# wuxiyang1996/iPLAN

Hardware: AMD Instinct MI355X
Metric: env-steps/sec (whole node), Hetero-Highway chaotic 5-agent (higher is better)
Workload: dtype f32; 1 GPU; Highway chaotic full iPLAN (Behaviour + GAT + soft update), 5 agents x 55 entities, 32 envs/GPU x 90 steps; step = 8 rollouts, each followed by insert + Behavior_policy.learn + Prediction_policy.learn, then IPPOLearner.train (15 epochs x 255 x 90 rows x 5 agents); envs_per_gpu=32

## Files before the change

### iplan_amd/csrc/ac_fwd_body.h

```cpp
#pragma once
#include "api_util.h"
#include "gru_tile.h"
#include "ac_kmap.h"

namespace iplan {

__device__ __forceinline__ f32x4 ac_act4(f32x4 v, bool tanh) {
    f32x4 r;
    for (int q = 0; q < 4; ++q) r[q] = tanh ? tanh_f(v[q]) : (v[q] > 0.0f ? v[q] : 0.0f);
    return r;
}

constexpr int AM = IPLAN_AC_HIDDEN;
constexpr int AT = AM / 16;
#ifndef AC_RT
#define AC_RT 2
#endif


template <int RT, int NW = 8>
struct AcShared {
#ifdef AC_NO_STAGED_TAIL
    static constexpr bool STAGED_BUILD = false, STAGED2 = false;
#else
    static constexpr bool STAGED_BUILD = RT == 1, STAGED2 = RT == 2;
#endif
    static constexpr int TLDW = AM + 8;
    static constexpr int TW_ROWS = STAGED2 ? AM + 3 * AM + 16 + 3 * AM : (STAGED_BUILD ? AM + 3 * AM + 16 : 0);
    static constexpr int TP_FLOATS = 912;
    float red[NW][16], red2[NW][16], cc[NW][2][AM];
    float hand[4];
    __attribute__((aligned(16))) f32x4 acc[RT == 1 ? 8 : 1][AT][64];
    __attribute__((aligned(16))) float tw[TW_ROWS ? TW_ROWS * TLDW : 4];
    __attribute__((aligned(16))) f32x4 gh[STAGED_BUILD ? 3 * AT : 1][64];
    __attribute__((aligned(16))) float tp[TW_ROWS ? TP_FLOATS : 4];
};

struct AcGrid {
    int bx, by, bz, gx, gy, gz;
};

struct AcProducers {
    int32_t* sync;
    int n_prod, n_cons;
};

__device__ __forceinline__ void ac_signal_producer_done(int32_t* sync) {
#ifdef IPLAN_HOST_EMULATION
    __syncthreads();
    if (threadIdx.x == 0) sync[0] += 1;
#else
    asm volatile("s_waitcnt vmcnt(0)" ::: "memory");
    __syncthreads();
    if (threadIdx.x == 0) {
#if IPLAN_FUSED_FENCES
        __builtin_amdgcn_fence(__ATOMIC_RELEASE, "agent");
#endif
        __hip_atomic_fetch_add(sync, 1, __ATOMIC_RELAXED, __HIP_MEMORY_SCOPE_AGENT);
    }
#endif
}

__device__ __forceinline__ void ac_wait_producers(const AcProducers& pr) {
#ifdef IPLAN_HOST_EMULATION
    if (threadIdx.x == 0) {
        if (pr.sync[0] < pr.n_prod) pr.sync[2] = 1;
        if (++pr.sync[1] == pr.n_cons) { pr.sync[0] = 0; pr.sync[1] = 0; }
    }
    __syncthreads();
#else
    if (threadIdx.x == 0) {
        int spins = 0;
        while (__hip_atomic_load(pr.sync, __ATOMIC_RELAXED, __HIP_MEMORY_SCOPE_AGENT) < pr.n_prod) {
            __builtin_amdgcn_s_sleep(2);
            if (++spins > (1 << 22)) { __hip_atomic_store(pr.sync + 2, 1, __ATOMIC_RELAXED, __HIP_MEMORY_SCOPE_AGENT); break; }
        }
#if IPLAN_FUSED_FENCES
        __builtin_amdgcn_fence(__ATOMIC_ACQUIRE, "agent");
#endif
        if (__hip_atomic_fetch_add(pr.sync + 1, 1, __ATOMIC_RELAXED, __HIP_MEMORY_SCOPE_AGENT) == pr.n_cons - 1) {
            __hip_atomic_store(pr.sync + 1, 0, __ATOMIC_RELAXED, __HIP_MEMORY_SCOPE_AGENT);
            __hip_atomic_store(pr.sync, 0, __ATOMIC_RELAXED, __HIP_MEMORY_SCOPE_AGENT);
        }
    }
    __syncthreads();
    asm volatile("" ::: "memory");
#endif
}

template <int RT, bool PRE, bool FUSED, int NW = 8>
__device__ __forceinline__ void ac_fwd_body(const IplanAcFwdArgs& a, const AcGrid& gp, AcShared<RT, NW>& sh, const AcProducers& prod) {
    auto& s_red = sh.red;
    auto& s_red2 = sh.red2;
    auto& s_cc = sh.cc;
    auto& s_acc = sh.acc;
    constexpr int TLDW = AM + 8;
#ifdef AC_NO_STAGED_TAIL
    constexpr bool STAGED_BUILD = false, STAGED2 = false;
#else
    constexpr bool STAGED_BUILD = RT == 1, STAGED2 = RT == 2;
#endif
    constexpr int TW_ROWS = AcShared<RT, NW>::TW_ROWS;
    static_assert(TLDW == AcShared<RT, NW>::TLDW, "tail weight row stride");
    auto& s_tw = sh.tw;
    auto& s_gh = sh.gh;
    constexpr int TP_FC1B = 0, TP_LN1W = 64, TP_LN1B = 128, TP_FC2B = 192, TP_LN2W = 256, TP_LN2B = 320, TP_BIH = 384, TP_BHH = 576,
                  TP_LN3W = 768, TP_LN3B = 832, TP_HEADB = 896, TP_FLOATS = 912;
    static_assert(TP_FLOATS == AcShared<RT, NW>::TP_FLOATS, "tail parameter vectors");
    auto& s_tp = sh.tp;

    int bx = gp.bx, by = gp.by, bz = gp.bz;
#ifndef AC_NO_XCD_REMAP
    {
        const int X = gp.gx, G = X * gp.gy * gp.gz;
        const int b = bx + X * (by + gp.gy * bz);
        const int k = b & 7, slot = b >> 3, q8 = G >> 3, r8 = G & 7;
        const int item = k * q8 + (k < r8 ? k : r8) + slot;
        bx = item % X;
        const int pair = item / X;
        by = pair % gp.gy;
        bz = pair / gp.gy;
    }
#endif
    const int net = by;
    const int which = a.which == 2 ? bz : a.which;
    const IplanAcNet& nw = which ? a.critic : a.actor;
    const float* __restrict__ P = nw.params + (int64_t)net * nw.params_s_net;
    const IplanAcFeatures& ft = a.feat;
    const int l = lane_id(), w = uniform_i(wave_id()), n = l & 15, g = l >> 4;
    const int ks = RT == 1 ? a.ksplit : 1;
    const int groups = NW / ks;
    const int part = w % ks;
    const int KW = (RT == 1 && !PRE && a.ksplit_wg > 1 && ks == 8) ? a.ksplit_wg : 1;
    const int pw = bx % KW;
    bx /= KW;
    const int kpart = part * KW + pw;
    const bool clk = !FUSED && a.phase_clocks && bx == 0 && by == 0 && bz == 0 && threadIdx.x == 0;
    if (clk) a.phase_clocks[0] = IPLAN_CLOCK();
    int64_t* fclk = (FUSED && a.phase_clocks && threadIdx.x == 0) ? a.phase_clocks + 8 * (gp.bx + gp.gx * (gp.by + gp.gy * gp.bz)) : nullptr;
    if (fclk) fclk[0] = IPLAN_CLOCK();
    const KMap km = make_kmap(ft);
    const int F = km.NW + km.n_actions + km.n_id;
    const int KT = km.kt0[4];
    const float* __restrict__ pkw = which ? a.packed_critic : a.packed_actor;
    if (pkw) pkw += (int64_t)net * a.packed_s_net;
    const float* __restrict__ pkg = pkw ? pkw + (int64_t)KT * 1024 : nullptr;
    const float* __restrict__ pkb = pkw ? pkg + (int64_t)KT * 16 : nullptr;
    const float* __restrict__ pkc = pkw ? pkb + (int64_t)KT * 16 : nullptr;
    const int T_lo = kpart, T_hi = KT, T_st = ks * KW;

    int rr[RT], last[RT];
    bool vld[RT];
    int64_t prr[RT];
    const float* src[RT][3];
    for (int t = 0; t < RT; ++t) {
        const int tile = (bx * groups + w / ks) * RT + t;
        rr[t] = tile * 16 + n;
        vld[t] = rr[t] < a.rows;
        prr[t] = vld[t] ? (int64_t)(rr[t] / ft.T) * ft.T_phys + (rr[t] % ft.T) : 0;
        for (int s = 0; s < 3; ++s)
            src[t][s] = ft.w[s] > 0 ? ft.src[s] + (int64_t)net * ft.s_net[s] + prr[t] * ft.s_row[s] : nullptr;
        last[t] = -1;
        if (vld[t] && ft.n_actions > 0) {
            if (ft.last_action) last[t] = ft.last_action[(int64_t)net * ft.la_s_net + prr[t] * ft.la_s_row];
            else if (ft.last_action64) last[t] = (int)ft.last_action64[(int64_t)net * ft.la64_s_net + prr[t] * ft.la64_s_row];
        }
    }

    const bool staged = STAGED_BUILD && ks == 8 && groups == 1 && a.saved == nullptr;
    if (STAGED_BUILD && staged) {
        const float* Wsrc[3] = {P + nw.off[IPLAN_AC_FC2_W], P + nw.off[IPLAN_AC_WIH], P + nw.off[IPLAN_AC_HEAD_W]};
        for (int c = (int)threadIdx.x; c < (AM + 3 * AM + 16) * 16; c += 64 * NW) {
            const int r = c >> 4, c4 = c & 15;
            f32x4 v = splat4(0.f);
            if (r < AM) v = *reinterpret_cast<const f32x4*>(Wsrc[0] + r * AM + 4 * c4);
            else if (r < 4 * AM) v = *reinterpret_cast<const f32x4*>(Wsrc[1] + (r - AM) * AM + 4 * c4);
            else if (r - 4 * AM < nw.n_out) v = *reinterpret_cast<const f32x4*>(Wsrc[2] + (r - 4 * AM) * AM + 4 * c4);
            *reinterpret_cast<f32x4*>(&s_tw[r * TLDW + 4 * c4]) = v;
        }
        const float* hsrc0 = which ? a.h_critic : a.h_actor;
        const float* hrow0 = hsrc0 + (int64_t)net * a.hs_net + prr[0] * a.hs_row;
        f32x4 h0[AT];
        for (int t = 0; t < AT; ++t) h0[t] = vload(hrow0, vld[0], AM, t);
        for (int t = w; t < 3 * AT; t += NW)
            s_gh[t][l] = dense_tile_ga<AT>(P + nw.off[IPLAN_AC_WHH], AM, 3 * AM, 16 * t, h0, bfrag_a(P + nw.off[IPLAN_AC_BHH], t));
    }

    if (STAGED2) {
        const float* Wsrc[4] = {P + nw.off[IPLAN_AC_FC2_W], P + nw.off[IPLAN_AC_WIH], P + nw.off[IPLAN_AC_HEAD_W], P + nw.off[IPLAN_AC_WHH]};
        for (int c = (int)threadIdx.x; c < TW_ROWS * 16; c += 64 * NW) {
            const int r = c >> 4, c4 = c & 15;
            f32x4 v = splat4(0.f);
            if (r < AM) v = *reinterpret_cast<const f32x4*>(Wsrc[0] + r * AM + 4 * c4);
            else if (r < 4 * AM) v = *reinterpret_cast<const f32x4*>(Wsrc[1] + (r - AM) * AM + 4 * c4);
            else if (r < 4 * AM + 16) { if (r - 4 * AM < nw.n_out) v = *reinterpret_cast<const f32x4*>(Wsrc[2] + (r - 4 * AM) * AM + 4 * c4); }
            else v = *reinterpret_cast<const f32x4*>(Wsrc[3] + (r - 4 * AM - 16) * AM + 4 * c4);
            *reinterpret_cast<f32x4*>(&s_tw[r * TLDW + 4 * c4]) = v;
        }
    }

    const bool lds_tail = STAGED2 || (STAGED_BUILD && staged);
    if (TW_ROWS && lds_tail) {
        const int tp_off[11] = {TP_FC1B, TP_LN1W, TP_LN1B, TP_FC2B, TP_LN2W, TP_LN2B, TP_BIH, TP_BHH, TP_LN3W, TP_LN3B, TP_HEADB};
        const int tp_src[11] = {IPLAN_AC_FC1_B, IPLAN_AC_LN1_W, IPLAN_AC_LN1_B, IPLAN_AC_FC2_B, IPLAN_AC_LN2_W, IPLAN_AC_LN2_B, IPLAN_AC_BIH,
                                IPLAN_AC_BHH, IPLAN_AC_LN3_W, IPLAN_AC_LN3_B, IPLAN_AC_HEAD_B};
#pragma unroll
        for (int k = 0; k < 11; ++k) {
            const int len = k == 10 ? 16 : ((k == 6 || k == 7) ? 3 * AM : AM), have = k == 10 ? nw.n_out : len;
            for (int i = (int)threadIdx.x; i < len; i += 64 * NW) s_tp[tp_off[k] + i] = i < have ? P[nw.off[tp_src[k]] + i] : 0.f;
        }
    }

    const bool fold = !PRE && RT == 1 && ks > 1 && a.ln_stats_mode == 0;
    float mu[RT], rstd[RT];
    float fsx = 0.f, fsxx = 0.f;
    float c1a[AT], c2a[AT];
    for (int o = 0; o < AT; ++o) { c1a[o] = 0.f; c2a[o] = 0.f; }
    if (fold) {
        for (int t = 0; t < RT; ++t) { mu[t] = 0.f; rstd[t] = 1.f; }
    } else if (PRE || a.ln_stats_mode == 2) {
        for (int t = 0; t < RT; ++t) {
            mu[t] = 0.f; rstd[t] = 0.f;
            if (vld[t]) {
                const float* st = a.ln_stats + (int64_t)net * a.ln_stats_s_net + prr[t] * 2;
                mu[t] = st[0]; rstd[t] = st[1];
            }
        }
    } else {
        float s[RT];
        for (int t = 0; t < RT; ++t) s[t] = 0.f;
        for (int T = T_lo; T < T_hi; T += T_st) {
            const KTile kt = ktile(km, T);
            for (int t = 0; t < RT; ++t) {
                const f32x4 x = kfeat<FUSED>(km, kt, src[t], vld[t], last[t], net);
                s[t] += (x[0] + x[1]) + (x[2] + x[3]);
            }
        }
        for (int t = 0; t < RT; ++t) s[t] = group_sum(s[t]);
        if (ks > 1) {
            if (g == 0) s_red[w][n] = s[0];
            __syncthreads();
            float m = 0.f;
            for (int p2 = 0; p2 < ks; ++p2) m += s_red[(w / ks) * ks + p2][n];
            s[0] = m;
            __syncthreads();
        }
        for (int t = 0; t < RT; ++t) mu[t] = s[t] / (float)F;
        float v2[RT];
        for (int t = 0; t < RT; ++t) v2[t] = 0.f;
        for (int T = T_lo; T < T_hi; T += T_st) {
            const KTile kt = ktile(km, T);
            for (int t = 0; t < RT; ++t) {
                const f32x4 x = kfeat<FUSED>(km, kt, src[t], vld[t], last[t], net);
                for (int q = 0; q < 4; ++q)
                    if (q < kt.nv) { const float d = x[q] - mu[t]; v2[t] = fmaf(d, d, v2[t]); }
            }
        }
        for (int t = 0; t < RT; ++t) v2[t] = group_sum(v2[t]);
        if (ks > 1) {
            if (g == 0) s_red[w][n] = v2[0];
            __syncthreads();
            float m = 0.f;
            for (int p2 = 0; p2 < ks; ++p2) m += s_red[(w / ks) * ks + p2][n];
            v2[0] = m;
        }
        for (int t = 0; t < RT; ++t) {
            rstd[t] = 1.0f / sqrtf(v2[t] / (float)F + 1e-5f);
            if (a.ln_stats_mode == 1 && vld[t] && g == 0 && part == 0) {
                float* st = a.ln_stats + (int64_t)net * a.ln_stats_s_net + prr[t] * 2;
                st[0] = mu[t]; st[1] = rstd[t];
            }
        }
    }

    if (clk) a.phase_clocks[1] = IPLAN_CLOCK();
    const float* fnw = P + nw.off[IPLAN_AC_FN_W];
    const float* fnb = P + nw.off[IPLAN_AC_FN_B];
    const float* W1 = P + nw.off[IPLAN_AC_FC1_W];
    f32x4 accs[RT][AT];
    for (int t = 0; t < RT; ++t)
        for (int o = 0; o < AT; ++o) accs[t][o] = splat4(0.f);
#ifdef AC_NO_GROUPS
    constexpr bool GROUPED = false;
#else
    constexpr bool GROUPED = !PRE && RT > 1;
#endif
    f32x4 blk[GROUPED ? RT : 1][GROUPED ? AT : 1];
    if (GROUPED)
        for (int t = 0; t < RT; ++t)
            for (int o = 0; o < AT; ++o) blk[GROUPED ? t : 0][GROUPED ? o : 0] = splat4(0.f);
    auto flush_group = [&]() {
        if constexpr (GROUPED)
            for (int t = 0; t < RT; ++t)
                for (int o = 0; o < AT; ++o) { accs[t][o] += blk[t][o]; blk[t][o] = splat4(0.f); }
    };
    auto acc_mma = [&](const f32x4& wfrag, const f32x4& xfrag, int t, int oo) {
        if constexpr (GROUPED) blk[t][oo] = mma_block(wfrag, xfrag, blk[t][oo]);
        else accs[t][oo] = mma_block(wfrag, xfrag, accs[t][oo]);
    };
    struct KOps {
        KTile kt;
        f32x4 gm, bt, x[RT], wf[AT];
    };
    auto kload = [&](int T, KOps& o) {
        o.kt = ktile(km, T);
        for (int t = 0; t < RT; ++t) o.x[t] = kfeat<FUSED>(km, o.kt, src[t], vld[t], last[t], net);
        if (pkw) {
            o.gm = *reinterpret_cast<const f32x4*>(pkg + T * 16 + 4 * g);
            o.bt = *reinterpret_cast<const f32x4*>(pkb + T * 16 + 4 * g);
            for (int oo = 0; oo < AT; ++oo) o.wf[oo] = *reinterpret_cast<const f32x4*>(pkw + ((int64_t)(T * AT + oo) * 64 + l) * 4);
            return;
        }
        o.gm = kcols(o.kt, fnw);
        o.bt = kcols(o.kt, fnb);
        for (int oo = 0; oo < AT; ++oo) o.wf[oo] = kcols(o.kt, W1 + (int64_t)(16 * oo + n) * F);
    };
    auto fold_mma = [&](const f32x4& x, const f32x4& gm, const f32x4& bt, const f32x4 (&wf)[AT], int nv) {
        f32x4 xg, gz, bz;
        for (int q = 0; q < 4; ++q) {
            const bool ok = q < nv;
            const float xv = (vld[0] && ok) ? x[q] : 0.f;
            xg[q] = ok ? xv * gm[q] : 0.f;
            fsx += xv;
            fsxx = fmaf(xv, xv, fsxx);
            gz[q] = ok ? gm[q] : 0.f;
            bz[q] = ok ? bt[q] : 0.f;
        }
        for (int oo = 0; oo < AT; ++oo) {
            accs[0][oo] = mma_block(wf[oo], xg, accs[0][oo]);
            if (!pkc)
                for (int q = 0; q < 4; ++q) {
                    c1a[oo] = fmaf(wf[oo][q], gz[q], c1a[oo]);
                    c2a[oo] = fmaf(wf[oo][q], bz[q], c2a[oo]);
                }
        }
    };
    auto kmma = [&](const KOps& o) {
        if (fold) { fold_mma(o.x[0], o.gm, o.bt, o.wf, o.kt.nv); return; }
        f32x4 xn[RT];
        for (int t = 0; t < RT; ++t)
            for (int q = 0; q < 4; ++q)
                xn[t][q] = (vld[t] && q < o.kt.nv) ? (o.x[t][q] - mu[t]) * rstd[t] * o.gm[q] + o.bt[q] : 0.f;
        for (int oo = 0; oo < AT; ++oo)
            for (int t = 0; t < RT; ++t) acc_mma(o.wf[oo], xn[t], t, oo);
    };
    struct FOps {
        f32x4 gm, bt, x[RT], wf[AT];
    };
    auto fload = [&](int T, int s, FOps& o) {
        const int f0 = 16 * (T - km.kt0[s]) + 4 * g;
        for (int t = 0; t < RT; ++t) o.x[t] = (FUSED && s > 0) ? coh_load16_untracked(src[t][s] + f0) : ldu4(src[t][s] + f0);
        if (pkw) {
            o.gm = *reinterpret_cast<const f32x4*>(pkg + T * 16 + 4 * g);
            o.bt = *reinterpret_cast<const f32x4*>(pkb + T * 16 + 4 * g);
            for (int oo = 0; oo < AT; ++oo) o.wf[oo] = *reinterpret_cast<const f32x4*>(pkw + ((int64_t)(T * AT + oo) * 64 + l) * 4);
            return;
        }
        const int wS = km.w[s];
        const int e = f0 / wS;
        const int c0 = e * km.W + km.off[s] + (f0 - e * wS);
        o.gm = ldu4(fnw + c0);
        o.bt = ldu4(fnb + c0);
        for (int oo = 0; oo < AT; ++oo) o.wf[oo] = ldu4(W1 + (int64_t)(16 * oo + n) * F + c0);
    };
    auto fmma = [&](const FOps& o) {
        f32x4 ox[RT];
        for (int t = 0; t < RT; ++t) ox[t] = FUSED ? after_load(o.x[t], o.wf[AT - 1][3]) : o.x[t];
        if (fold) { fold_mma(ox[0], o.gm, o.bt, o.wf, 4); return; }
        f32x4 xn[RT];
        for (int t = 0; t < RT; ++t)
            for (int q = 0; q < 4; ++q) xn[t][q] = vld[t] ? (ox[t][q] - mu[t]) * rstd[t] * o.gm[q] + o.bt[q] : 0.f;
        for (int oo = 0; oo < AT; ++oo)
            for (int t = 0; t < RT; ++t) acc_mma(o.wf[oo], xn[t], t, oo);
    };
#ifndef AC_PF
#define AC_PF 2
#endif
#ifndef AC_GROUP_ROUNDS
#define AC_GROUP_ROUNDS 3
#endif
#ifndef AC_PF1
#define AC_PF1 3
#endif
    constexpr int PF = RT == 1 ? AC_PF1 : AC_PF;
    if (PRE) {
        for (int t = 0; t < RT; ++t) {
            const float* zrow = a.fc1_pre + (((int64_t)which * a.n_agents + net) * a.rows + (vld[t] ? rr[t] : 0)) * AM;
            for (int o = 0; o < AT; ++o) accs[t][o] = vload_a(zrow, vld[t], o);
            const int64_t zpart = 2 * (int64_t)a.n_agents * a.rows * AM;
            for (int pp = 1; pp < a.fc1_pre_parts; ++pp)
                for (int o = 0; o < AT; ++o) accs[t][o] += vload_a(zrow + pp * zpart, vld[t], o);
        }
    }
    for (int s = 0; s < (PRE ? 0 : 4); ++s) {
        if (FUSED && s == 1) {
            if (fclk) fclk[1] = IPLAN_CLOCK();
            ac_wait_producers(prod);
            if (fclk) fclk[2] = IPLAN_CLOCK();
        }
        const int kt0s = uniform_i(km.kt0[s]);
        const int b_end = imin(T_hi, uniform_i(km.kt0[s + 1]));
        const int b_lo = kt0s + ((kpart - kt0s) % T_st + T_st) % T_st;
        if (b_lo >= b_end) continue;
        int f_hi = b_lo;
        if (s < 3 && (uniform_i(km.w[s]) & 3) == 0 && uniform_i(ft.w[s]) > 0) f_hi = imin(b_end, kt0s + uniform_i(km.len[s]) / 16);
        int T_slow = b_lo;
        if (f_hi > b_lo) {
            FOps ring[PF];
            int T = b_lo;
            if (b_lo + (2 * PF - 1) * T_st < f_hi) {
                for (int i = 0; i < PF; ++i) fload(b_lo + i * T_st, s, ring[i]);
                IPLAN_SCHED_FENCE();
                int rounds = 0;
                for (; T + (2 * PF - 1) * T_st < f_hi; T += PF * T_st) {
                    for (int i = 0; i < PF; ++i) {
                        fmma(ring[i]);
                        IPLAN_SCHED_FENCE();
                        fload(T + (i + PF) * T_st, s, ring[i]);
                        IPLAN_SCHED_FENCE();
                    }
                    if (GROUPED && ++rounds == AC_GROUP_ROUNDS) { flush_group(); rounds = 0; }
                }
            } else {
                for (int i = 0; i < PF; ++i)
                    if (b_lo + i * T_st < f_hi) fload(b_lo + i * T_st, s, ring[i]);
            }
            IPLAN_SCHED_FENCE();
            for (; T < f_hi; T += PF * T_st) {
                for (int i = 0; i < PF; ++i) {
                    if (T + i * T_st < f_hi) {
                        fmma(ring[i]);
                        IPLAN_SCHED_FENCE();
                        if (T + (i + PF) * T_st < f_hi) fload(T + (i + PF) * T_st, s, ring[i]);
                        IPLAN_SCHED_FENCE();
                    }
                }
            }
            T_slow = b_lo + ((f_hi - b_lo + T_st - 1) / T_st) * T_st;
#if !defined(IPLAN_HOST_EMULATION)
            if (FUSED) asm volatile("s_waitcnt vmcnt(0)" ::: "memory");
#endif
        }
        for (int T = T_slow; T < b_end; T += T_st) {
            KOps o;
            kload(T, o);
            kmma(o);
        }
        flush_group();
    }
    if (fclk) fclk[3] = IPLAN_CLOCK();
    if (ks > 1) {
        for (int t = 0; t < AT; ++t) s_acc[w][t][l] = accs[0][t];
        if (fold) {
            fsx = group_sum(fsx);
            fsxx = group_sum(fsxx);
            if (g == 0) { s_red[w][n] = fsx; s_red2[w][n] = fsxx; }
            if (!pkc)
                for (int t = 0; t < AT; ++t) {
                    const float c1 = group_sum(c1a[t]), c2 = group_sum(c2a[t]);
                    if (g == 0) { s_cc[w][0][16 * t + n] = c1; s_cc[w][1][16 * t + n] = c2; }
                }
        }
        __syncthreads();
        if (part == 0) {
            for (int t = 0; t < AT; ++t) {
                f32x4 sum = s_acc[w][t][l];
                for (int p2 = 1; p2 < ks; ++p2) sum += s_acc[w + p2][t][l];
                accs[0][t] = sum;
            }
        }
        if (fold) {
            if (part == 0) {
                float sx = 0.f, sxx = 0.f;
                for (int p2 = 0; p2 < ks; ++p2) { sx += s_red[w + p2][n]; sxx += s_red2[w + p2][n]; }
                if (KW > 1) {
                    const int unit = (bz * gp.gy + by) * (gp.gx / KW) + bx;
                    float* slot = a.ks_scratch + ((int64_t)unit * KW + pw) * IPLAN_AC_KS_SLOT_FLOATS;
                    for (int t = 0; t < AT; ++t) coh_store16(slot + (t * 64 + l) * 4, accs[0][t]);
                    if (g == 0) { coh_store(slot + AT * 256 + n, sx); coh_store(slot + AT * 256 + 16 + n, sxx); }
                    int ticket = 0;
#ifdef IPLAN_HOST_EMULATION
                    IPLAN_WAVE_SYNC();
                    if (l == 0) { ticket = a.ks_count[unit]; a.ks_count[unit] = ticket + 1 == KW ? 0 : ticket + 1; s_red[0][0] = (float)ticket; }
                    IPLAN_WAVE_SYNC();
                    ticket = (int)s_red[0][0];
#else
#if IPLAN_FUSED_FENCES
                    __builtin_amdgcn_fence(__ATOMIC_RELEASE, "agent");
                    if (l == 0) ticket = __hip_atomic_fetch_add(a.ks_count + unit, 1, __ATOMIC_ACQ_REL, __HIP_MEMORY_SCOPE_AGENT);
#else
                    asm volatile("s_waitcnt vmcnt(0)" ::: "memory");
                    if (l == 0) ticket = __hip_atomic_fetch_add(a.ks_count + unit, 1, __ATOMIC_RELAXED, __HIP_MEMORY_SCOPE_AGENT);
#endif
                    ticket = __builtin_amdgcn_readfirstlane(ticket);
#endif
                    if (ticket != KW - 1) {
                        if (STAGED_BUILD && staged) {
                            if (l == 0) sh.hand[0] = 0.f;
#ifndef IPLAN_HOST_EMULATION
                            asm volatile("s_waitcnt lgkmcnt(0)" ::: "memory");
#endif
                        }
                        return;
                    }
#ifndef IPLAN_HOST_EMULATION
                    if (l == 0) __hip_atomic_store(a.ks_count + unit, 0, __ATOMIC_RELAXED, __HIP_MEMORY_SCOPE_AGENT);
#if IPLAN_FUSED_FENCES
                    __builtin_amdgcn_fence(__ATOMIC_ACQUIRE, "agent");
#endif
#endif
                    sx = 0.f; sxx = 0.f;
                    for (int t = 0; t < AT; ++t) accs[0][t] = splat4(0.f);
                    for (int q2 = 0; q2 < KW; ++q2) {
                        const float* sl = a.ks_scratch + ((int64_t)unit * KW + q2) * IPLAN_AC_KS_SLOT_FLOATS;
                        f32x4 pt[AT];
                        for (int t = 0; t < AT; ++t) pt[t] = coh_load16_untracked(sl + (t * 64 + l) * 4);
                        const float psx = coh_load(sl + AT * 256 + n), psxx = coh_load(sl + AT * 256 + 16 + n);
                        for (int t = 0; t < AT; ++t) accs[0][t] += after_load(pt[t], psxx);
                        sx += psx;
                        sxx += psxx;
                    }
                }
                mu[0] = sx / (float)F;
                rstd[0] = 1.0f / sqrtf(fmaxf(sxx / (float)F - mu[0] * mu[0], 0.f) + 1e-5f);
                for (int t = 0; t < AT; ++t)
                    for (int q = 0; q < 4; ++q) {
                        const int o = 16 * t + 4 * g + q;
                        float c1 = 0.f, c2 = 0.f;
                        if (pkc) { c1 = pkc[o]; c2 = pkc[AM + o]; }
                        else for (int p2 = 0; p2 < ks; ++p2) { c1 += s_cc[w + p2][0][o]; c2 += s_cc[w + p2][1][o]; }
                        accs[0][t][q] = rstd[0] * (accs[0][t][q] - mu[0] * c1) + c2;
                    }
            }
        }
    }
    if (clk) a.phase_clocks[2] = IPLAN_CLOCK();
    if (fclk) fclk[4] = IPLAN_CLOCK();
    if (STAGED2) __syncthreads();
    const bool ptail = STAGED_BUILD && staged;
    if (STAGED_BUILD && ptail) {
        if (part == 0) {
            for (int t = 0; t < AT; ++t) s_acc[0][t][l] = accs[0][t];
            if (l == 0) sh.hand[0] = 1.f;
        }
        __syncthreads();
        if (sh.hand[0] == 0.f || w >= AT) return;
        for (int t = 0; t < AT; ++t) accs[0][t] = s_acc[0][t][l];
    } else if (part != 0) return;

  const bool act_tanh = a.act_tanh != 0;
  for (int rt = 0; rt < RT; ++rt) {
    const int r = rr[rt];
    const bool valid = vld[rt];
    const int64_t pr = prr[rt];
    const float mu_ = mu[rt], rstd_ = rstd[rt];
    f32x4 acc[AT];
    for (int t = 0; t < AT; ++t) acc[t] = accs[rt][t];
    if (RT > 1 && (r - n) >= a.rows) break;
    float* sv = a.saved ? a.saved + (((int64_t)which * a.n_agents + net) * a.rows + (valid ? r : 0)) * IPLAN_AC_SAVE_FLOATS : nullptr;
    float mu1 = 0.f, rs1 = 0.f, mu2 = 0.f, rs2 = 0.f, mu3, rs3;
    auto pv = [&](int tp, int which_vec, int t) { return (TW_ROWS && lds_tail) ? bfrag_a(s_tp + tp, t) : bfrag_a(P + nw.off[which_vec], t); };
    const float* hsrc = which ? a.h_critic : a.h_actor;
    const float* hrow = hsrc + (int64_t)net * a.hs_net + pr * a.hs_row;
    f32x4 h[AT], hnew[AT];
    f32x4 f[AT], gmv[AT], btv[AT];
    if (STAGED_BUILD && ptail) {
        const f32x4 hw = vload(hrow, valid, AM, w);
        for (int t = 0; t < AT; ++t) f[t] = ac_act4(acc[t] + bfrag_a(s_tp + TP_FC1B, t), act_tanh);
        for (int t = 0; t < AT; ++t) { gmv[t] = bfrag_a(s_tp + TP_LN1W, t); btv[t] = bfrag_a(s_tp + TP_LN1B, t); }
        layer_norm_tiles_f<AT>(f, gmv, btv, &mu1, &rs1);
        s_acc[RT == 1 ? 1 : 0][w][l] = ac_act4(dense_tile<AT>(s_tw, TLDW, 16 * w, f, bfrag_a(s_tp + TP_FC2B, w)), act_tanh);
        __syncthreads();
        f32x4 f2p[AT];
        for (int t = 0; t < AT; ++t) f2p[t] = s_acc[RT == 1 ? 1 : 0][t][l];
        for (int t = 0; t < AT; ++t) { gmv[t] = bfrag_a(s_tp + TP_LN2W, t); btv[t] = bfrag_a(s_tp + TP_LN2B, t); }
        layer_norm_tiles_f<AT>(f2p, gmv, btv, &mu2, &rs2);
        const float* sWi = s_tw + AM * TLDW;
        const f32x4 pr_s = dense_tile<AT>(sWi, TLDW, 16 * w, f2p, bfrag_a(s_tp + TP_BIH, w) + s_gh[w][l]);
        const f32x4 pz_s = dense_tile<AT>(sWi, TLDW, AM + 16 * w, f2p, bfrag_a(s_tp + TP_BIH, AT + w) + s_gh[AT + w][l]);
        const f32x4 gn_s = dense_tile<AT>(sWi, TLDW, 2 * AM + 16 * w, f2p, bfrag_a(s_tp + TP_BIH, 2 * AT + w));
        s_acc[RT == 1 ? 2 : 0][w][l] = gru_gates(pr_s, pz_s, gn_s, s_gh[2 * AT + w][l], hw).h;
        __syncthreads();
        if (w != 0) return;
        for (int t = 0; t < AT; ++t) hnew[t] = s_acc[RT == 1 ? 2 : 0][t][l];
    } else {
    for (int t = 0; t < AT; ++t) h[t] = vload(hrow, valid, AM, t);
    for (int t = 0; t < AT; ++t) {
        f[t] = ac_act4(acc[t] + pv(TP_FC1B, IPLAN_AC_FC1_B, t), act_tanh);
        if (sv) vstore(sv, valid, AM, t, f[t]);
    }
    for (int t = 0; t < AT; ++t) { gmv[t] = pv(TP_LN1W, IPLAN_AC_LN1_W, t); btv[t] = pv(TP_LN1B, IPLAN_AC_LN1_B, t); }
    layer_norm_tiles_f<AT>(f, gmv, btv, &mu1, &rs1);
    if (sv) for (int t = 0; t < AT; ++t) vstore(sv + AM, valid, AM, t, f[t]);
    f32x4 f2[AT];
    for (int t = 0; t < AT; ++t) {
        if (lds_tail) f2[t] = ac_act4(dense_tile<AT>(s_tw, TLDW, 16 * t, f, pv(TP_FC2B, IPLAN_AC_FC2_B, t)), act_tanh);
        else f2[t] = ac_act4(dense_tile_ga<AT>(P + nw.off[IPLAN_AC_FC2_W], AM, AM, 16 * t, f, bfrag_a(P + nw.off[IPLAN_AC_FC2_B], t)), act_tanh);
        if (sv) vstore(sv + 2 * AM, valid, AM, t, f2[t]);
    }
    for (int t = 0; t < AT; ++t) { gmv[t] = pv(TP_LN2W, IPLAN_AC_LN2_W, t); btv[t] = pv(TP_LN2B, IPLAN_AC_LN2_B, t); }
    layer_norm_tiles_f<AT>(f2, gmv, btv, &mu2, &rs2);
    if (sv) for (int t = 0; t < AT; ++t) vstore(sv + 3 * AM, valid, AM, t, f2[t]);
    {
        const float* Wi = P + nw.off[IPLAN_AC_WIH];
        const float* Wh = P + nw.off[IPLAN_AC_WHH];
        for (int t = 0; t < AT; ++t) {
            if (STAGED_BUILD && staged) {
                const float* sWi = s_tw + AM * TLDW;
                const f32x4 pr_s = dense_tile<AT>(sWi, TLDW, 16 * t, f2, bfrag_a(s_tp + TP_BIH, t) + s_gh[t][l]);
                const f32x4 pz_s = dense_tile<AT>(sWi, TLDW, AM + 16 * t, f2, bfrag_a(s_tp + TP_BIH, AT + t) + s_gh[AT + t][l]);
                const f32x4 gn_s = dense_tile<AT>(sWi, TLDW, 2 * AM + 16 * t, f2, bfrag_a(s_tp + TP_BIH, 2 * AT + t));
                hnew[t] = gru_gates(pr_s, pz_s, gn_s, s_gh[2 * AT + t][l], h[t]).h;
                continue;
            }
            f32x4 prr = pv(TP_BIH, IPLAN_AC_BIH, t) + pv(TP_BHH, IPLAN_AC_BHH, t);
            f32x4 pz = pv(TP_BIH, IPLAN_AC_BIH, AT + t) + pv(TP_BHH, IPLAN_AC_BHH, AT + t);
            f32x4 gn = pv(TP_BIH, IPLAN_AC_BIH, 2 * AT + t);
            f32x4 hn = pv(TP_BHH, IPLAN_AC_BHH, 2 * AT + t);
            if (STAGED2) {
                const float* sWi = s_tw + AM * TLDW;
                const float* sWh = s_tw + (4 * AM + 16) * TLDW;
                prr = dense_tile<AT>(sWh, TLDW, 16 * t, h, dense_tile<AT>(sWi, TLDW, 16 * t, f2, prr));
                pz = dense_tile<AT>(sWh, TLDW, AM + 16 * t, h, dense_tile<AT>(sWi, TLDW, AM + 16 * t, f2, pz));
                gn = dense_tile<AT>(sWi, TLDW, 2 * AM + 16 * t, f2, gn);
                hn = dense_tile<AT>(sWh, TLDW, 2 * AM + 16 * t, h, hn);
            } else {
            prr = dense_tile_ga<AT>(Wi, AM, 3 * AM, 16 * t, f2, prr);
            prr = dense_tile_ga<AT>(Wh, AM, 3 * AM, 16 * t, h, prr);
            pz = dense_tile_ga<AT>(Wi, AM, 3 * AM, AM + 16 * t, f2, pz);
            pz = dense_tile_ga<AT>(Wh, AM, 3 * AM, AM + 16 * t, h, pz);
            gn = dense_tile_ga<AT>(Wi, AM, 3 * AM, 2 * AM + 16 * t, f2, gn);
            hn = dense_tile_ga<AT>(Wh, AM, 3 * AM, 2 * AM + 16 * t, h, hn);
            }
            const GruGates o = gru_gates(prr, pz, gn, hn, h[t]);
            hnew[t] = o.h;
            if (sv) {
                vstore(sv + 4 * AM, valid, AM, t, o.r);
                vstore(sv + 5 * AM, valid, AM, t, o.z);
                vstore(sv + 6 * AM, valid, AM, t, o.n);
                vstore(sv + 7 * AM, valid, AM, t, o.hn);
                vstore(sv + 8 * AM, valid, AM, t, o.h);
            }
        }
    }
    }
    float* hout = which ? a.h_critic_out : a.h_actor_out;
    if (hout) {
        float* orow = a.ho_s_row ? hout + (int64_t)net * a.ho_s_net + (int64_t)(valid ? r : 0) * a.ho_s_row
                                 : hout + ((int64_t)net * a.rows + (valid ? r : 0)) * AM;
        for (int t = 0; t < AT; ++t) vstore(orow, valid, AM, t, hnew[t]);
    }
    for (int t = 0; t < AT; ++t) { gmv[t] = pv(TP_LN3W, IPLAN_AC_LN3_W, t); btv[t] = pv(TP_LN3B, IPLAN_AC_LN3_B, t); }
    layer_norm_tiles_f<AT>(hnew, gmv, btv, &mu3, &rs3);
    if (sv) {
        for (int t = 0; t < AT; ++t) vstore(sv + 9 * AM, valid, AM, t, hnew[t]);
        if (valid && g == 0) {
            float* st = sv + 10 * AM;
            st[0] = mu_; st[1] = rstd_; st[2] = mu1; st[3] = rs1; st[4] = mu2; st[5] = rs2; st[6] = mu3; st[7] = rs3;
        }
    }
    const int n_out = nw.n_out;
    const f32x4 lg = lds_tail
        ? dense_tile<AT>(s_tw + 4 * AM * TLDW, TLDW, 0, hnew, bfrag_a(s_tp + TP_HEADB, 0))
        : dense_tile_ga<AT>(P + nw.off[IPLAN_AC_HEAD_W], AM, n_out, 0, hnew, bfrag(P + nw.off[IPLAN_AC_HEAD_B], n_out, 0));
    const int64_t orow = (int64_t)net * a.rows + (valid ? r : 0);
    if (which == 1) {
        if (valid && g == 0 && a.values) a.values[orow] = lg[0];
        continue;
    }
    f32x4 x;
    float m = -INFINITY;
    for (int q = 0; q < 4; ++q) {
        const int idx = 4 * g + q;
        x[q] = lg[q];
        if (idx < n_out) {
            if (a.avail && valid && a.avail[(int64_t)net * a.av_s_net + pr * a.av_s_row + idx] == 0) x[q] = -1e10f;
            m = fmaxf(m, x[q]);
        }
    }
    m = fmaxf(m, __shfl_xor(m, 16));
    m = fmaxf(m, __shfl_xor(m, 32));
    f32x4 e;
    float se = 0.f;
    for (int q = 0; q < 4; ++q) { e[q] = (4 * g + q < n_out) ? expf(x[q] - m) : 0.f; se += e[q]; }
    se = group_sum(se);
    const float lse = m + logf(se);
    f32x4 lp, pb;
    for (int q = 0; q < 4; ++q) { lp[q] = x[q] - lse; pb[q] = e[q] / se; }
    int action = 0;
    if (a.mode == 2) {
        action = valid ? (int)a.actions_in[(int64_t)net * a.act_s_net + pr * a.act_s_row] : 0;
    } else {
        f32x4 key;
        float best = -INFINITY;
        for (int q = 0; q < 4; ++q) {
            const int idx = 4 * g + q;
            key[q] = -INFINITY;
            if (idx < n_out) {
                key[q] = pb[q];
                if (a.mode == 1) key[q] = pb[q] / a.q_noise[orow * n_out + idx];
                best = fmaxf(best, key[q]);
            }
        }
        best = fmaxf(best, __shfl_xor(best, 16));
        best = fmaxf(best, __shfl_xor(best, 32));
        int cand = 1 << 30;
        for (int q = 3; q >= 0; --q)
            if (4 * g + q < n_out && key[q] == best) cand = 4 * g + q;
        int o = __shfl_xor(cand, 16); cand = o < cand ? o : cand;
        o = __shfl_xor(cand, 32); cand = o < cand ? o : cand;
        action = cand;
        if (valid && g == 0 && a.actions_out) {
            if (a.ao_s_row) a.actions_out[(int64_t)net * a.ao_s_net + (int64_t)r * a.ao_s_row] = (int64_t)action;
            else a.actions_out[orow] = (int64_t)action;
        }
        if (valid && a.onehot_out)
            for (int q = 0; q < 4; ++q)
                if (4 * g + q < n_out) a.onehot_out[(int64_t)net * a.oh_s_net + (int64_t)r * a.oh_s_row + 4 * g + q] = (4 * g + q == action) ? 1.0f : 0.0f;
    }
    float sel = 0.f, ent = 0.f;
    for (int q = 0; q < 4; ++q) {
        const int idx = 4 * g + q;
        if (idx < n_out) {
            if (idx == action) sel += lp[q];
            ent -= pb[q] * lp[q];
            if (a.probs && valid) a.probs[orow * n_out + idx] = pb[q];
        }
    }
    sel = group_sum(sel);
    ent = group_sum(ent);
    if (valid && g == 0) {
        if (a.logp) a.logp[orow] = sel;
        if (a.entropy) a.entropy[orow] = ent;
    }
  }
    if (clk) a.phase_clocks[3] = IPLAN_CLOCK();
    if (fclk) fclk[5] = IPLAN_CLOCK();
}

}
```

### iplan_amd/csrc/wave_tile.h

```cpp
#pragma once
#include <hip/hip_runtime.h>

typedef float f32x4 __attribute__((ext_vector_type(4)));

#ifdef IPLAN_HOST_EMULATION
#define IPLAN_DYN_LDS(name) float* name = iplan_emu::dyn_lds()
#else
#define IPLAN_DYN_LDS(name) extern __shared__ __attribute__((aligned(16))) float name[]
#endif

#ifdef IPLAN_HOST_EMULATION
#define IPLAN_CLOCK() ((int64_t)0)
#else
#define IPLAN_CLOCK() ((int64_t)wall_clock64())
#endif
#ifdef IPLAN_HOST_EMULATION
#define IPLAN_SCHED_FENCE() do {} while (0)
#define IPLAN_WAVE_SYNC() iplan_emu::wave_sync()
#else
#define IPLAN_SCHED_FENCE() __builtin_amdgcn_sched_barrier(0)
#define IPLAN_WAVE_SYNC() __builtin_amdgcn_wave_barrier()
#endif

#ifdef IPLAN_HOST_EMULATION
#define IPLAN_LDS_BARRIER() __syncthreads()
#else
#define IPLAN_LDS_BARRIER() asm volatile("s_waitcnt lgkmcnt(0)\n\ts_barrier" ::: "memory")
#endif

namespace iplan {

#ifdef IPLAN_HOST_EMULATION
#define IPLAN_TILE_SYNC(cnt, target) __syncthreads()
#else
__device__ __forceinline__ void iplan_tile_sync(int* cnt, int target) {
    asm volatile("s_waitcnt lgkmcnt(0)" ::: "memory");
    if ((threadIdx.x & 63u) == 0) __hip_atomic_fetch_add(cnt, 1, __ATOMIC_RELAXED, __HIP_MEMORY_SCOPE_WORKGROUP);
    while (__hip_atomic_load(cnt, __ATOMIC_RELAXED, __HIP_MEMORY_SCOPE_WORKGROUP) < target) __builtin_amdgcn_s_sleep(1);
    asm volatile("" ::: "memory");
}
#define IPLAN_TILE_SYNC(cnt, target) iplan_tile_sync((cnt), (target))
#endif

__device__ __forceinline__ int lane_id() { return (int)(threadIdx.x & 63u); }
__device__ __forceinline__ int wave_id() { return (int)(threadIdx.x >> 6); }

__host__ __device__ __forceinline__ int imin(int a, int b) { return a < b ? a : b; }
__host__ __device__ __forceinline__ int imax(int a, int b) { return a > b ? a : b; }

__device__ __forceinline__ f32x4 mfma4(float a, float b, f32x4 c) {
    return __builtin_amdgcn_mfma_f32_16x16x4f32(a, b, c, 0, 0, 0);
}

typedef __bf16 bf16x8 __attribute__((ext_vector_type(8)));
struct Bf3 {
    bf16x8 p0, p1, p2;
};
__device__ __forceinline__ Bf3 split_bf3_scalar(f32x4 lo, f32x4 hi) {
    Bf3 s;
    for (int j = 0; j < 8; ++j) {
        const float v = j < 4 ? lo[j] : hi[j - 4];
        const __bf16 b0 = (__bf16)v;
        const float r1 = v - (float)b0;
        const __bf16 b1 = (__bf16)r1;
        const float r2 = r1 - (float)b1;
        s.p0[j] = b0;
        s.p1[j] = b1;
        s.p2[j] = (__bf16)r2;
    }
    return s;
}
typedef float f32x2 __attribute__((ext_vector_type(2)));
typedef __bf16 bf16x2 __attribute__((ext_vector_type(2)));
typedef uint32_t u32x4 __attribute__((ext_vector_type(4)));
typedef uint32_t u32x2 __attribute__((ext_vector_type(2)));
__device__ __forceinline__ uint32_t bf16_pack2(f32x2 v) {
    return __builtin_bit_cast(uint32_t, __builtin_convertvector(v, bf16x2));
}
__device__ __forceinline__ f32x2 bf16_unpack2(uint32_t u) {
    f32x2 r;
    r[0] = __builtin_bit_cast(float, u << 16);
    r[1] = __builtin_bit_cast(float, u & 0xffff0000u);
    return r;
}
__device__ __forceinline__ void split_bf3_pair(f32x2 v, uint32_t& q0, uint32_t& q1, uint32_t& q2) {
    q0 = bf16_pack2(v);
    const f32x2 r1 = v - bf16_unpack2(q0);
    q1 = bf16_pack2(r1);
    const f32x2 r2 = r1 - bf16_unpack2(q1);
    q2 = bf16_pack2(r2);
}
__device__ __forceinline__ Bf3 split_bf3_pairs(f32x4 lo, f32x4 hi) {
    u32x4 q0, q1, q2;
    for (int k = 0; k < 4; ++k) {
        f32x2 v;
        v[0] = k < 2 ? lo[2 * k] : hi[2 * k - 4];
        v[1] = k < 2 ? lo[2 * k + 1] : hi[2 * k - 3];
        uint32_t a, b, c;
        split_bf3_pair(v, a, b, c);
        q0[k] = a; q1[k] = b; q2[k] = c;
    }
    Bf3 s;
    s.p0 = __builtin_bit_cast(bf16x8, q0);
    s.p1 = __builtin_bit_cast(bf16x8, q1);
    s.p2 = __builtin_bit_cast(bf16x8, q2);
    return s;
}
__device__ __forceinline__ Bf3 split_bf3(f32x4 lo, f32x4 hi) {
#ifdef IPLAN_SPLIT_PAIRS
    return split_bf3_pairs(lo, hi);
#else
    return split_bf3_scalar(lo, hi);
#endif
}
__device__ __forceinline__ f32x4 mfma_bf16(bf16x8 a, bf16x8 b, f32x4 c) {
    return __builtin_amdgcn_mfma_f32_16x16x32_bf16(a, b, c, 0, 0, 0);
}
__device__ __forceinline__ Bf3 wfrag_bf3(const float* __restrict__ W, int ld, int rows, int o0, int k0) {
    const int l = lane_id();
    const int r = o0 + (l & 15);
    const int rc = r < rows ? r : rows - 1;
    const float* p = W + (size_t)rc * ld + k0 + 4 * (l >> 4);
    f32x4 lo = *reinterpret_cast<const f32x4*>(p), hi = *reinterpret_cast<const f32x4*>(p + 16);
    if (r >= rows) lo = hi = f32x4{0.f, 0.f, 0.f, 0.f};
    return split_bf3(lo, hi);
}

__device__ __forceinline__ Bf3 wfrag_bf3_scaled(const float* __restrict__ W, int ld, int rows, int o0, int k0, float c) {
    const int l = lane_id();
    const int r = o0 + (l & 15);
    const int rc = r < rows ? r : rows - 1;
    const float* p = W + (size_t)rc * ld + k0 + 4 * (l >> 4);
    f32x4 lo = *reinterpret_cast<const f32x4*>(p), hi = *reinterpret_cast<const f32x4*>(p + 16);
    if (r >= rows) lo = hi = f32x4{0.f, 0.f, 0.f, 0.f};
    return split_bf3(lo * c, hi * c);
}

__device__ __forceinline__ Bf3 wfrag_t_bf3(const float* __restrict__ W, int ld, int o0, int k0) {
    const int l = lane_id();
    const float* p = W + (size_t)(k0 + 4 * (l >> 4)) * ld + o0 + (l & 15);
    f32x4 lo, hi;
    for (int j = 0; j < 4; ++j) { lo[j] = p[(size_t)j * ld]; hi[j] = p[(size_t)(16 + j) * ld]; }
    return split_bf3(lo, hi);
}

__device__ __forceinline__ f32x4 splat4(float v) {
    f32x4 r = {v, v, v, v};
    return r;
}

#ifdef IPLAN_EXACT_GATES
__device__ __forceinline__ float sigmoid_f(float x) { return 1.0f / (1.0f + expf(-x)); }
__device__ __forceinline__ float tanh_f(float x) { return tanhf(x); }
#else
__device__ __forceinline__ float sigmoid_f(float x) {
    return __builtin_amdgcn_rcpf(1.0f + __builtin_amdgcn_exp2f(-1.4426950408889634f * x));
}
__device__ __forceinline__ float tanh_f(float x) {
    return 1.0f - 2.0f * __builtin_amdgcn_rcpf(__builtin_amdgcn_exp2f(2.8853900817779268f * x) + 1.0f);
}
#endif

__device__ __forceinline__ f32x4 relu4(f32x4 v) {
    f32x4 r;
    for (int q = 0; q < 4; ++q) r[q] = v[q] > 0.0f ? v[q] : 0.0f;
    return r;
}

__device__ __forceinline__ f32x4 wfrag(const float* __restrict__ W, int ld, int rows, int cols,
                                       int o0, int k0) {
    const int l = lane_id();
    const int r = o0 + (l & 15);
    const int c = k0 + 4 * (l >> 4);
    f32x4 v = {0.f, 0.f, 0.f, 0.f};
    if (r < rows) {
        const float* p = W + (size_t)r * ld + c;
        if (c + 3 < cols && ((ld & 3) == 0) && ((((size_t)p) & 15) == 0)) {
            v = *reinterpret_cast<const f32x4*>(p);
        } else {
            for (int q = 0; q < 4; ++q)
                if (c + q < cols) v[q] = p[q];
        }
    }
    return v;
}

__device__ __forceinline__ f32x4 wfrag_a(const float* __restrict__ W, int ld, int rows, int o0, int k0) {
    const int l = lane_id();
    const int r = o0 + (l & 15);
    const int rc = r < rows ? r : rows - 1;
    f32x4 v = *reinterpret_cast<const f32x4*>(W + (size_t)rc * ld + k0 + 4 * (l >> 4));
    if (r >= rows) v = f32x4{0.f, 0.f, 0.f, 0.f};
    return v;
}

__device__ __forceinline__ f32x4 wfrag_ta(const float* __restrict__ W, int ld, int o0, int k0) {
    const int l = lane_id();
    const float* p = W + (size_t)(k0 + 4 * (l >> 4)) * ld + o0 + (l & 15);
    f32x4 v;
    v[0] = p[0]; v[1] = p[ld]; v[2] = p[2 * ld]; v[3] = p[3 * ld];
    return v;
}

__device__ __forceinline__ f32x4 bfrag_a(const float* __restrict__ b, int t) {
    return *reinterpret_cast<const f32x4*>(b + 16 * t + 4 * (lane_id() >> 4));
}

__device__ __forceinline__ f32x4 wfrag_t(const float* __restrict__ W, int ld, int rows, int cols,
                                         int o0, int k0) {
    const int l = lane_id();
    const int c = o0 + (l & 15);
    const int r = k0 + 4 * (l >> 4);
    f32x4 v = {0.f, 0.f, 0.f, 0.f};
    if (c < cols)
        for (int q = 0; q < 4; ++q)
            if (r + q < rows) v[q] = W[(size_t)(r + q) * ld + c];
    return v;
}

__device__ __forceinline__ f32x4 bfrag(const float* __restrict__ b, int dim, int t) {
    const int c = 16 * t + 4 * (lane_id() >> 4);
    f32x4 v = {0.f, 0.f, 0.f, 0.f};
    for (int q = 0; q < 4; ++q)
        if (c + q < dim) v[q] = b[c + q];
    return v;
}

#ifdef IPLAN_HOST_EMULATION
#define IPLAN_GLOBAL_AS
#else
#define IPLAN_GLOBAL_AS __attribute__((address_space(1)))
#endif
template <class T>
__device__ __forceinline__ const IPLAN_GLOBAL_AS T* as_global(const T* p) { return (const IPLAN_GLOBAL_AS T*)p; }

__device__ __forceinline__ float keep_if(bool ok, float v) {
    return __builtin_bit_cast(float, __builtin_bit_cast(uint32_t, v) & (ok ? 0xFFFFFFFFu : 0u));
}
__device__ __forceinline__ f32x4 zero_unless(bool ok, f32x4 v) {
    const uint32_t m = ok ? 0xFFFFFFFFu : 0u;
    f32x4 r;
    for (int q = 0; q < 4; ++q) r[q] = __builtin_bit_cast(float, __builtin_bit_cast(uint32_t, (float)v[q]) & m);
    return r;
}
__device__ __forceinline__ int uniform_i(int v) {
#ifdef IPLAN_HOST_EMULATION
    return v;
#else
    return __builtin_amdgcn_readfirstlane(v);
#endif
}

__device__ __forceinline__ f32x4 vload(const float* __restrict__ row, bool valid, int dim, int t) {
    const int c = 16 * t + 4 * (lane_id() >> 4);
    f32x4 v = {0.f, 0.f, 0.f, 0.f};
    if (valid) {
        if (c + 3 < dim && ((((size_t)(row + c)) & 15) == 0)) {
            v = *reinterpret_cast<const f32x4*>(row + c);
        } else {
            for (int q = 0; q < 4; ++q)
                if (c + q < dim) v[q] = row[c + q];
        }
    }
    return v;
}

__device__ __forceinline__ void vstore(float* __restrict__ row, bool valid, int dim, int t, f32x4 v) {
    const int c = 16 * t + 4 * (lane_id() >> 4);
    if (valid) {
        if (c + 3 < dim && ((((size_t)(row + c)) & 15) == 0)) {
            *reinterpret_cast<f32x4*>(row + c) = v;
        } else {
            for (int q = 0; q < 4; ++q)
                if (c + q < dim) row[c + q] = v[q];
        }
    }
}

#ifndef IPLAN_FUSED_FENCES
#define IPLAN_FUSED_FENCES 0
#endif
__device__ __forceinline__ void coh_store(float* p, float v) {
#if defined(IPLAN_HOST_EMULATION) || IPLAN_FUSED_FENCES
    *p = v;
#else
    __hip_atomic_store(p, v, __ATOMIC_RELAXED, __HIP_MEMORY_SCOPE_AGENT);
#endif
}
__device__ __forceinline__ float coh_load(const float* p) {
#if defined(IPLAN_HOST_EMULATION) || IPLAN_FUSED_FENCES
    return *p;
#else
    return __hip_atomic_load(as_global(p), __ATOMIC_RELAXED, __HIP_MEMORY_SCOPE_AGENT);
#endif
}
__device__ __forceinline__ f32x4 coh_load16_untracked(const float* p) {
#if defined(IPLAN_HOST_EMULATION) || IPLAN_FUSED_FENCES
    return *reinterpret_cast<const f32x4*>(p);
#else
    f32x4 v;
    asm volatile("global_load_dwordx4 %0, %1, off sc1" : "=v"(v) : "v"(p) : "memory");
    return v;
#endif
}
__device__ __forceinline__ void coh_store16(float* p, f32x4 v) {
#if defined(IPLAN_HOST_EMULATION) || IPLAN_FUSED_FENCES
    *reinterpret_cast<f32x4*>(p) = v;
#else
    asm volatile("global_store_dwordx4 %0, %1, off sc1" ::"v"(p), "v"(v) : "memory");
#endif
}
__device__ __forceinline__ f32x4 after_load(f32x4 v, float dep) {
#if !defined(IPLAN_HOST_EMULATION)
    asm volatile("" : "+v"(v) : "v"(dep));
#endif
    return v;
}
template <bool COH>
__device__ __forceinline__ void vstore_c(float* __restrict__ row, bool valid, int dim, int t, f32x4 v) {
    if (!COH) { vstore(row, valid, dim, t, v); return; }
    const int c = 16 * t + 4 * (lane_id() >> 4);
    if (valid) {
        if (c + 3 < dim && ((((size_t)(row + c)) & 15) == 0)) {
            coh_store16(row + c, v);
        } else {
            for (int q = 0; q < 4; ++q)
                if (c + q < dim) coh_store(row + c + q, v[q]);
        }
    }
}

__device__ __forceinline__ f32x4 vload_a(const float* __restrict__ row, bool valid, int t) {
    f32x4 v = {0.f, 0.f, 0.f, 0.f};
    if (valid) v = *reinterpret_cast<const f32x4*>(row + 16 * t + 4 * (lane_id() >> 4));
    return v;
}
__device__ __forceinline__ void vstore_a(float* __restrict__ row, bool valid, int t, f32x4 v) {
    if (valid) *reinterpret_cast<f32x4*>(row + 16 * t + 4 * (lane_id() >> 4)) = v;
}

__device__ __forceinline__ f32x4 mma_block(f32x4 w, f32x4 x, f32x4 acc) {
    acc = mfma4(w[0], x[0], acc);
    acc = mfma4(w[1], x[1], acc);
    acc = mfma4(w[2], x[2], acc);
    acc = mfma4(w[3], x[3], acc);
    return acc;
}

__device__ __forceinline__ float group_sum(float v) {
    v += __shfl_xor(v, 16);
    v += __shfl_xor(v, 32);
    return v;
}

__device__ __forceinline__ float wave_sum(float v) {
    for (int m = 1; m < 64; m <<= 1) v += __shfl_xor(v, m);
    return v;
}
__device__ __forceinline__ float wave_max(float v) {
    for (int m = 1; m < 64; m <<= 1) v = fmaxf(v, __shfl_xor(v, m));
    return v;
}

struct GruGates {
    f32x4 r, z, n, hn, h;
};
__device__ __forceinline__ GruGates gru_gates(f32x4 pre_r, f32x4 pre_z, f32x4 gi_n, f32x4 gh_n, f32x4 h_prev) {
    GruGates o;
    for (int q = 0; q < 4; ++q) {
        o.r[q] = sigmoid_f(pre_r[q]);
        o.z[q] = sigmoid_f(pre_z[q]);
        o.hn[q] = gh_n[q];
        o.n[q] = tanh_f(gi_n[q] + o.r[q] * gh_n[q]);
        o.h[q] = (1.0f - o.z[q]) * o.n[q] + o.z[q] * h_prev[q];
    }
    return o;
}

__device__ __forceinline__ GruGates gru_gates_folded(f32x4 pre_r, f32x4 pre_z, f32x4 gi_n, f32x4 gh_n, f32x4 h_prev) {
    GruGates o;
    for (int q = 0; q < 4; ++q) {
#ifdef IPLAN_EXACT_GATES
        o.r[q] = 1.0f / (1.0f + exp2f(pre_r[q]));
        o.z[q] = 1.0f / (1.0f + exp2f(pre_z[q]));
        o.n[q] = 1.0f - 2.0f / (exp2f(gi_n[q] + o.r[q] * gh_n[q]) + 1.0f);
#else
        o.r[q] = __builtin_amdgcn_rcpf(1.0f + __builtin_amdgcn_exp2f(pre_r[q]));
        o.z[q] = __builtin_amdgcn_rcpf(1.0f + __builtin_amdgcn_exp2f(pre_z[q]));
        o.n[q] = 1.0f - 2.0f * __builtin_amdgcn_rcpf(__builtin_amdgcn_exp2f(gi_n[q] + o.r[q] * gh_n[q]) + 1.0f);
#endif
        o.hn[q] = gh_n[q];
        o.h[q] = (1.0f - o.z[q]) * o.n[q] + o.z[q] * h_prev[q];
    }
    return o;
}

}
```

Baseline: 90870 env-steps/s.

## Prefetch fold weights for first k-blocks before waiting on producers in fused AC kernel

In the fused actor-critic forward with RT==1, the weight tiles for the first few fold k-blocks of stages 1 and 2 (up to AC_HOLD) are loaded into registers before the producer wait. After the wait, only the activations and gamma values are fetched for those blocks, and the normal contraction loop resumes past them. A vmcnt drain is added at ring entry, and after_load now uses explicit v_movs so the dependency ordering holds. The aim is to hide weight-load latency behind the producer spin wait, at the cost of more held vector registers and extra control logic.

```diff
diff --git a/iplan_amd/csrc/ac_fwd_body.h b/iplan_amd/csrc/ac_fwd_body.h
--- a/iplan_amd/csrc/ac_fwd_body.h
+++ b/iplan_amd/csrc/ac_fwd_body.h
@@ -392,15 +392,25 @@
                 for (int o = 0; o < AT; ++o) accs[t][o] += vload_a(zrow + pp * zpart, vld[t], o);
         }
     }
-    for (int s = 0; s < (PRE ? 0 : 4); ++s) {
-        if (FUSED && s == 1) {
-            if (fclk) fclk[1] = IPLAN_CLOCK();
-            ac_wait_producers(prod);
-            if (fclk) fclk[2] = IPLAN_CLOCK();
-        }
+#ifndef AC_HOLD
+#define AC_HOLD 5
+#endif
+    constexpr bool HOLDS = FUSED && RT == 1 && !PRE;
+    constexpr int HOLD = HOLDS ? AC_HOLD : 1;
+    f32x4 hwf[HOLD][AT], hgm[HOLD], hx[HOLD];
+    int h_T[HOLD], h_f0[HOLD];
+    int nh1 = 0, nh = 0;
+#if defined(IPLAN_HOST_EMULATION)
+#define IPLAN_RING_ENTRY_DRAIN() do {} while (0)
+#else
+#define IPLAN_RING_ENTRY_DRAIN() do { if (FUSED && s > 0) asm volatile("s_waitcnt vmcnt(0)" ::: "memory"); } while (0)
+#endif
+    auto contract_blocks = [&](int s_lo, int s_hi) {
+    for (int s = s_lo; s < s_hi; ++s) {
         const int kt0s = uniform_i(km.kt0[s]);
         const int b_end = imin(T_hi, uniform_i(km.kt0[s + 1]));
-        const int b_lo = kt0s + ((kpart - kt0s) % T_st + T_st) % T_st;
+        const int held = HOLDS ? (s == 1 ? nh1 : (s == 2 ? nh - nh1 : 0)) : 0;
+        const int b_lo = kt0s + ((kpart - kt0s) % T_st + T_st) % T_st + held * T_st;
         if (b_lo >= b_end) continue;
         int f_hi = b_lo;
         if (s < 3 && (uniform_i(km.w[s]) & 3) == 0 && uniform_i(ft.w[s]) > 0) f_hi = imin(b_end, kt0s + uniform_i(km.len[s]) / 16);
@@ -409,6 +419,7 @@
             FOps ring[PF];
             int T = b_lo;
             if (b_lo + (2 * PF - 1) * T_st < f_hi) {
+                IPLAN_RING_ENTRY_DRAIN();
                 for (int i = 0; i < PF; ++i) fload(b_lo + i * T_st, s, ring[i]);
                 IPLAN_SCHED_FENCE();
                 int rounds = 0;
@@ -422,6 +433,7 @@
                     if (GROUPED && ++rounds == AC_GROUP_ROUNDS) { flush_group(); rounds = 0; }
                 }
             } else {
+                IPLAN_RING_ENTRY_DRAIN();
                 for (int i = 0; i < PF; ++i)
                     if (b_lo + i * T_st < f_hi) fload(b_lo + i * T_st, s, ring[i]);
             }
@@ -447,6 +459,63 @@
             kmma(o);
         }
         flush_group();
+    }
+    };
+#undef IPLAN_RING_ENTRY_DRAIN
+    static_assert(!(FUSED && PRE), "the fused launch contracts its own rows");
+    if constexpr (!FUSED) {
+        contract_blocks(0, PRE ? 0 : 4);
+    } else {
+        contract_blocks(0, 1);
+        if constexpr (HOLDS) {
+            if (fold && pkw && pkc) {
+                int h_lo[2], h_n[2];
+                for (int s2 = 1; s2 <= 2; ++s2) {
+                    const int k0 = uniform_i(km.kt0[s2]), lo = k0 + ((kpart - k0) % T_st + T_st) % T_st;
+                    int hi = lo;
+                    if ((uniform_i(km.w[s2]) & 3) == 0 && uniform_i(ft.w[s2]) > 0) hi = imin(imin(T_hi, uniform_i(km.kt0[s2 + 1])), k0 + uniform_i(km.len[s2]) / 16);
+                    h_lo[s2 - 1] = lo;
+                    h_n[s2 - 1] = hi > lo ? (hi - lo + T_st - 1) / T_st : 0;
+                }
+                nh1 = imin(HOLD, h_n[0]);
+                nh = nh1;
+                if (nh1 == h_n[0] && h_lo[0] + h_n[0] * T_st >= imin(T_hi, uniform_i(km.kt0[2]))) nh += imin(HOLD - nh1, h_n[1]);
+                if (nh > 0) {
+                    for (int i = 0; i < HOLD; ++i) {
+                        const int j = i < nh ? i : 0;
+                        const int T = j < nh1 ? h_lo[0] + j * T_st : h_lo[1] + (j - nh1) * T_st;
+                        h_f0[i] = 16 * (T - (j < nh1 ? uniform_i(km.kt0[1]) : uniform_i(km.kt0[2])));
+                        h_T[i] = T;
+                        for (int oo = 0; oo < AT; ++oo) hwf[i][oo] = *reinterpret_cast<const f32x4*>(pkw + ((int64_t)(T * AT + oo) * 64 + l) * 4);
+                    }
+#ifndef IPLAN_HOST_EMULATION
+                    for (int i = 0; i < HOLD; ++i)
+                        for (int oo = 0; oo < AT; ++oo) asm volatile("" : "+v"(hwf[i][oo]));
+#endif
+                }
+            }
+        }
+        if (fclk) fclk[1] = IPLAN_CLOCK();
+        ac_wait_producers(prod);
+        if (fclk) fclk[2] = IPLAN_CLOCK();
+        if constexpr (HOLDS) {
+            if (nh > 0) {
+                for (int i = 0; i < HOLD; ++i)
+                    hx[i] = coh_load16_untracked(((i < nh ? i : 0) < nh1 ? src[0][1] : src[0][2]) + h_f0[i] + 4 * g);
+                for (int i = 0; i < HOLD; ++i) {
+                    int go = h_T[i] * 16 + 4 * g;
+#ifndef IPLAN_HOST_EMULATION
+                    asm volatile("" : "+v"(go));
+#endif
+                    hgm[i] = *reinterpret_cast<const f32x4*>(pkg + go);
+                }
+                for (int i = 0; i < HOLD; ++i) {
+                    const f32x4 ox = after_load(hx[i], hgm[i][3]);
+                    if (i < nh) fold_mma(ox, hgm[i], hgm[i] , hwf[i], 4);
+                }
+            }
+        }
+        contract_blocks(1, 4);
     }
     if (fclk) fclk[3] = IPLAN_CLOCK();
     if (ks > 1) {
diff --git a/iplan_amd/csrc/wave_tile.h b/iplan_amd/csrc/wave_tile.h
--- a/iplan_amd/csrc/wave_tile.h
+++ b/iplan_amd/csrc/wave_tile.h
@@ -312,7 +312,11 @@
 }
 __device__ __forceinline__ f32x4 after_load(f32x4 v, float dep) {
 #if !defined(IPLAN_HOST_EMULATION)
-    asm volatile("" : "+v"(v) : "v"(dep));
+    float r0, r1, r2, r3;
+    asm volatile("v_mov_b32 %0, %4\n\tv_mov_b32 %1, %5\n\tv_mov_b32 %2, %6\n\tv_mov_b32 %3, %7"
+                 : "=&v"(r0), "=&v"(r1), "=&v"(r2), "=&v"(r3)
+                 : "v"((float)v[0]), "v"((float)v[1]), "v"((float)v[2]), "v"((float)v[3]), "v"(dep));
+    v = f32x4{r0, r1, r2, r3};
 #endif
     return v;
 }
```

Result: no change. 90370 env-steps/s (-0.6%).
